# thourihan/DeepfakeDetection

Hardware: AMD Instinct MI355X
Metric: train images/sec @224^2 (EfficientNet-B0) (higher is better)
Workload: dtype bf16; 1 GPU; EfficientNet-b0 (timm flavour) 224x224 train step: bf16 fwd + label-smoothed CE + bwd + AdamW, random-init weights, 2 classes; per_gpu_batch=256, global_batch=256, parallelism=dp1, launch=hipgraph

## Files before the change

deepfakedetection_amd/_lib.py:

```python

from __future__ import annotations

import ctypes
from ctypes import POINTER, Structure, c_double, c_float, c_int, c_int64, c_long, c_size_t, c_uint32, c_void_p
from pathlib import Path

import os as _os

LIB_PATH = Path(_os.environ.get("DFD_LIB_PATH") or Path(__file__).resolve().parent / "libdfd_hip.so")

DFD_OK = 0
ERRORS = {-1: "DFD_EINVAL", -2: "DFD_EUNSUPPORTED", -3: "DFD_ELAUNCH", -4: "DFD_EWORKSPACE"}
F32, BF16 = 0, 1
ACT_NONE, ACT_SILU, ACT_RELU, ACT_GELU = 0, 1, 2, 3
PRO_NONE, PRO_BN_ACT, PRO_BN_ACT_GATE, PRO_AFFINE2 = 0, 1, 2, 3
MAX_PARTIALS = 1024
ADAMW_TABLE_COLS = 5
ADAMW_HP_LEN = 8
EMA_TABLE_COLS = 4
EMA_LERP, EMA_COPY = 0, 1
CLIP_MODE_NORM, CLIP_MODE_VALUE = 0, 1
CLIP_CFG_LEN = 2
CLIP_STATE_LEN = 8
(CLIP_NORM, CLIP_COEF, CLIP_SKIP, CLIP_STEPS, CLIP_CLIPPED, CLIP_SKIPPED, CLIP_NORM_SUM, CLIP_NORM_MAX) = range(8)
# ... 28 lines not shown


class StemShape(Structure):
    _fields_ = [(n, c_int) for n in ("N", "H", "W", "Cout", "Ho", "Wo", "k", "stride", "pad_top", "pad_left")]


class Mat(Structure):

    _fields_ = [(n, c_long) for n in ("sb", "sh", "sr", "sc")]


class Prologue(Structure):
    _fields_ = [
        ("mode", c_int), ("act", c_int), ("HW", c_int), ("_pad", c_int),
        ("a2", c_void_p), ("coef", c_void_p), ("gate", c_void_p),
    ]


P = c_void_p
_PI = POINTER(c_int)

SIGNATURES: dict[str, tuple] = {
    "dfd_version": (c_int, []),
    "dfd_tune": (c_int, [c_int, c_int]),
    "dfd_dw_mm_plan": (c_int, [POINTER(DwShape), c_int, _PI]),
    "dfd_bn_finalize": (c_int, [P, c_int, c_int, c_double, P, P, P, P, c_float, c_float, P, P]),
    "dfd_bn_eval_coeffs": (c_int, [P, P, P, P, c_float, c_int, P, P]),
    "dfd_bn_bwd_finalize": (c_int, [P, c_int, c_int, c_double, P, P, c_int, P, P, c_int, P, P]),
    "dfd_bn_act_apply": (c_int, [c_int, P, P, c_int, P, P, P, c_int, c_int, c_int, P]),
    "dfd_bn_bwd_reduce": (c_int, [c_int, P, P, P, P, c_int, c_int, c_int, P, c_int, _PI, P]),
    "dfd_gemm_bias_act": (c_int, [c_int, P, P, c_int, c_int, c_int, P, c_int, P, P, c_int, P, P, P]),
    "dfd_gemm_plan": (c_int, [c_int, c_int, c_int]),
    "dfd_pw_ntd_plan": (c_int, [c_int, c_int, c_int]),
    "dfd_bias_grad_ws": (c_size_t, [c_int, c_int, c_int]),
    "dfd_bias_grad": (c_int, [c_int, P, P, c_int, c_int, c_int, P, c_int, P, c_size_t, P]),
    "dfd_act_bn_bwd": (c_int, [c_int, P, P, P, P, P, c_int, P, c_int, c_int, c_int, P, c_int, _PI, P]),
    "dfd_act_bn_bwd_se": (c_int, [c_int, P, P, P, P, P, c_int, P, c_int, c_int, c_int, P, c_int, _PI, P, P, c_int, P, P, P, P, c_int, P]),
    "dfd_prep_weights_multi": (c_int, [P, c_int, P]),
    "dfd_resize_crop_u8": (c_int, [P, P, P, c_int, c_int, c_int, c_int, P]),
    "dfd_augment_u8": (c_int, [P, P, P, c_int, c_int, c_int, P]),
    "dfd_image_prep": (c_int, [P, P, c_int, c_int, c_int, POINTER(c_float), POINTER(c_float), P, P, P]),
    "dfd_pool_ws": (c_size_t, [c_int, c_int, c_int, c_int]),
    "dfd_pool_act": (c_int, [c_int, P, P, c_int, P, c_int, c_int, c_int, P, c_size_t, P]),
    "dfd_pool_bwd_reduce": (c_int, [c_int, P, P, P, c_int, P, c_int, c_int, c_int, P, c_size_t, P]),
    "dfd_scale_rows": (c_int, [c_int, P, P, P, c_int, c_int, c_int, P]),
    "dfd_se_fc_fwd": (c_int, [P, P, P, P, P, c_int, c_int, c_int, c_int, P, P, P, P]),
    "dfd_se_fc_bwd": (c_int, [P, P, P, P, P, P, c_int, c_int, c_int, c_int, P, P, P, P, P, c_int, P, P]),
    "dfd_dwconv_fwd": (c_int, [c_int, P, P, c_int, P, P, POINTER(DwShape), P, c_int, _PI, P]),
# ... 176 lines not shown
```

deepfakedetection_amd/csrc/dfd_pw.h:

```cpp
#pragma once
#include "dfd_common.h"
#include <type_traits>

typedef __attribute__((ext_vector_type(8))) __bf16 bf16x8_t;
typedef __attribute__((ext_vector_type(4))) short short4_t;
typedef __attribute__((ext_vector_type(8))) short short8_t;
typedef __attribute__((ext_vector_type(4))) float f32x4_t;

#define PW_BM 128

struct ProArgs {
    const void* a2;
    const float* coef;
    const float* gate;
    int HW;
    unsigned hw_magic;
    int hw_shift;
};
__device__ __forceinline__ int pro_image(const ProArgs& pa, int m) {
    return pa.hw_shift < 0 ? m : (int)(__umulhi((unsigned)m, pa.hw_magic) >> pa.hw_shift);
}

struct Magic { unsigned mul; int sh; };
static inline Magic make_magic(int d) {
    Magic m{0u, -1};
    if (d > 1) {
        int s = 0;
        while ((1ll << s) < d) ++s;
        m.mul = (unsigned)(((1ull << (31 + s)) + (unsigned long long)d - 1) / (unsigned long long)d);
        m.sh = s - 1;
    }
    return m;
// ... 104 lines not shown
        case DFD_ACT_SILU: { constexpr int ACT = DFD_ACT_SILU; __VA_ARGS__; } break; \
        case DFD_ACT_GELU: { constexpr int ACT = DFD_ACT_GELU; __VA_ARGS__; } break; \
        default: return DFD_EUNSUPPORTED;                                            \
    }
static inline bool pro_ok(const dfd_prologue* p) {
    if (!p) return true;
    switch (p->mode) {
        case DFD_PRO_NONE: return true;
        case DFD_PRO_BN_ACT: return p->coef != nullptr;
        case DFD_PRO_BN_ACT_GATE: return p->coef && p->gate && p->HW > 0;
        case DFD_PRO_AFFINE2: return p->coef && p->a2;
        default: return false;
    }
}
static inline ProArgs pro_args(const dfd_prologue* p) {
    ProArgs a{nullptr, nullptr, nullptr, 1, 0u, -1};
    if (p) { a.a2 = p->a2; a.coef = p->coef; a.gate = p->gate; a.HW = p->HW > 0 ? p->HW : 1; }
    if (a.HW > 1) {
        int sh = 0;
        while ((1ll << sh) < a.HW) ++sh;
        a.hw_magic = (unsigned)(((1ull << (31 + sh)) + (unsigned long long)a.HW - 1) / (unsigned long long)a.HW);
        a.hw_shift = sh - 1;
    }
    return a;
}


__device__ __forceinline__ int tn_off_bf16(int m, int ch) {
    const int f = ((m & 3) | (((m >> 3) & 1) << 2)) << 1;
    return m * 256 + ((ch ^ f) << 4);
}

// ... 18 lines not shown
```

deepfakedetection_amd/csrc/dfd_pwconv.hip:

```cpp
#include "dfd_pw.h"

template <typename T, int BN, int BM> struct NtLds {
    static constexpr int A_BYTES = BM * 128;
    static constexpr int B_BYTES = BN * 128;
    static constexpr int OROW = BN * (int)sizeof(T) + 16;
    static constexpr int OBYTES = BM * OROW;
    static constexpr int BOFF = ((2 * A_BYTES > OBYTES ? 2 * A_BYTES : OBYTES) + 15) / 16 * 16;
    static constexpr int TOTAL = BOFF + 2 * B_BYTES;
};

template <typename T, int BN, int BM, int PRO, int ACT, bool RES, bool STATS, bool CONV = false, int EACT = -1>
__global__ void __launch_bounds__(DFD_THREADS, 2)
k_pw_nt(const T* __restrict__ a, ProArgs pa, const T* __restrict__ w, T* __restrict__ out, const T* __restrict__ res,
        int M, int K, int Nout, int m_tiles, int n_tiles, int gx, float* __restrict__ partials, ConvArgs cv,
        const float* __restrict__ ebn = nullptr) {
    constexpr int E = El<T>::EPC;
    constexpr int BK = El<T>::BK;
    constexpr int NTW = BN / 32;
    using L = NtLds<T, BN, BM>;
    constexpr int RF = BM / 32;
    constexpr int AI = BM / 32;
    constexpr int OROW = L::OROW;
    extern __shared__ __attribute__((aligned(16))) unsigned char smem[];

// ... 771 lines not shown
    const bool small = ((M + 127) / 128) * ((Cout + 127) / 128) < 256;
#define CONV_GO(TT, BNV) return small ? conv_nt_launch<TT, BNV, 64>(x, s, in_bnstate, in_act, w_nk, y, Cout, partials, pcap, nparts, st) \
                                      : conv_nt_launch<TT, BNV, 128>(x, s, in_bnstate, in_act, w_nk, y, Cout, partials, pcap, nparts, st)
    if (dtype == DFD_BF16) { if (Cout <= 64) CONV_GO(bf16, 64); CONV_GO(bf16, 128); }
    if (dtype == DFD_F32) { if (Cout <= 64) CONV_GO(float, 64); CONV_GO(float, 128); }
#undef CONV_GO
    return DFD_EINVAL;
}

extern "C" int dfd_pwconv_fwd(int dtype, const void* a, const dfd_prologue* pro, const void* w, void* out,
                              const void* residual, int M, int K, int Nout, float* partials, int pcap, int* nparts,
                              dfd_stream stream) {
    if (!a || !w || !out || M < 1 || K < 8 || Nout < 8 || K % 8 || Nout % 8 || !pro_ok(pro)) return DFD_EINVAL;
    if (partials && (!nparts || pcap < 1)) return DFD_EINVAL;
    hipStream_t st = (hipStream_t)stream;
    const int rc = dfd_pw_ntw(dtype, a, pro, w, out, residual, M, K, Nout, partials, pcap, nparts, st);
    if (rc != DFD_EUNSUPPORTED) return rc;
    if (dtype == DFD_BF16 && !(!pro && !residual && !partials && dfd_gemm_plan(M, K, Nout))) {
        const int rd = dfd_pw_ntd(dtype, a, pro, w, out, residual, M, K, Nout, partials, pcap, nparts, st);
        if (rd != DFD_EUNSUPPORTED) return rd;
    }
    if (dtype == DFD_BF16) return pw_nt_t<bf16>(a, pro, w, out, residual, M, K, Nout, partials, pcap, nparts, st);
    if (dtype == DFD_F32) return pw_nt_t<float>(a, pro, w, out, residual, M, K, Nout, partials, pcap, nparts, st);
    return DFD_EINVAL;
}

extern "C" int dfd_pwconv_fwd_eval(int dtype, const void* a, const void* w, const float* out_bnstate, int out_act, void* out,
                                   int M, int K, int Nout, dfd_stream stream) {
    if (!a || !w || !out || !out_bnstate || M < 1 || K < 8 || Nout < 8 || K % 8 || Nout % 8) return DFD_EINVAL;
    hipStream_t st = (hipStream_t)stream;
// ... 148 lines not shown
```

deepfakedetection_amd/csrc/dfd_pwntd.hip:

```cpp
#include "dfd_pw.h"
#include "dfd_dwm.h"

#define ND_BM 64
#define ND_RED_BYTES (DFD_THREADS * 16 * 4)
#define ND_MAXN 192
#define ND_MINT 16

typedef __attribute__((address_space(3))) unsigned char nd_lds_u8;

__device__ __forceinline__ void nd_dma16(const void* src, unsigned lds_addr) {
    asm volatile("s_mov_b32 m0, %1\n\ts_nop 0\n\tglobal_load_lds_dwordx4 %0, off" : : "v"(src), "s"(lds_addr) : "memory");
}
template <int N> __device__ __forceinline__ void nd_wait_vm() { asm volatile("s_waitcnt vmcnt(%0)" : : "n"(N) : "memory"); }
__device__ __forceinline__ unsigned nd_lds_addr(const void* p) {
    return (unsigned)reinterpret_cast<uintptr_t>((nd_lds_u8*)p);
}

template <int NT, int PRO> struct NdGeom {
    static constexpr int BN = 16 * NT;
    static constexpr int WPC = (2 * NT + 3) / 4;
    static constexpr int JA = PRO == DFD_PRO_AFFINE2 ? 4 : 2;
    static constexpr int J = JA + WPC;
    static constexpr int WOFF = JA * 4096;
    static constexpr int STAGE = WOFF + WPC * 4096;
// ... 196 lines not shown
        float* red = reinterpret_cast<float*>(smem + (4 * 16 * OROW + 15) / 16 * 16);
        if (lact) {
            float* p = red + ((wave * RL + er) * CPR + ec) * 16;
            store_f32<8>(p, s1);
            store_f32<8>(p + 8, s2);
        }
        __syncthreads();
        for (int idx = t; idx < CPR * 16; idx += DFD_THREADS) {
            const int c = idx >> 4, x = idx & 15;
            float s = 0.f;
#pragma unroll 4
            for (int r = 0; r < 4 * RL; ++r) s += red[(r * CPR + c) * 16 + x];
            const int col = n0 + c * 8 + (x & 7);
            if (col < Nout) partials[(long)mt * 2 * Nout + (x >> 3) * Nout + col] = s;
        }
    }
}

template <int NT, int PRO, int ACT, bool RES, bool STATS>
static int ntd_launch(const void* a, const ProArgs& pa, const void* w, void* out, const void* residual, int M, int K, int Nout,
                      float* partials, int imgs, hipStream_t st) {
    using G = NdGeom<NT, PRO>;
    constexpr int NROW = PRO == DFD_PRO_AFFINE2 ? 3 : 2;
    const int m_tiles = (M + ND_BM - 1) / ND_BM, n_tiles = (Nout + G::BN - 1) / G::BN;
    const int nk = (K + 63) / 64;
    const int ctab = PRO == DFD_PRO_NONE ? 0 : (NROW * K * 4 + 1023) / 1024 * 1024 + 256;
    const int gtab = PRO == DFD_PRO_BN_ACT_GATE ? (imgs * K * 4 + 1023) / 1024 * 1024 + 256 : 0;
    const int tables = ctab + gtab;
    int ns;
    const int half = 80 * 1024 - 512;
// ... 34 lines not shown
    if (rc == DFD_OK && stats) *nparts = (M + ND_BM - 1) / ND_BM;
    return rc;
}

static int ntd_pick(int Nout) {
    const int tiles = (Nout + ND_MAXN - 1) / ND_MAXN;
    const int per = ((Nout + tiles - 1) / tiles + 15) / 16;
    return per <= 4 ? 4 : per <= 6 ? 6 : per <= 8 ? 8 : 12;
}

static bool ntd_serves(int M, int K, int cap) {
    const int m_tiles = (M + ND_BM - 1) / ND_BM;
    return (dfd_tune_get(DFD_TUNE_PW_NTD) & 1) && m_tiles >= ND_MINT && m_tiles <= cap && K >= 64 && (long)M * K < (1l << 30);
}

int dfd_pw_ntd(int dtype, const void* a, const dfd_prologue* pro, const void* w, void* out, const void* residual, int M, int K,
               int Nout, float* partials, int pcap, int* nparts, hipStream_t st) {
    const int cap = partials ? (pcap < DFD_MAX_PARTIALS ? pcap : DFD_MAX_PARTIALS) : DFD_MAX_PARTIALS;
    if (dtype != DFD_BF16 || !ntd_serves(M, K, cap)) return DFD_EUNSUPPORTED;
    switch (ntd_pick(Nout)) {
        case 4: return ntd_nt<4>(a, pro, w, out, residual, M, K, Nout, partials, nparts, st);
        case 6: return ntd_nt<6>(a, pro, w, out, residual, M, K, Nout, partials, nparts, st);
        case 8: return ntd_nt<8>(a, pro, w, out, residual, M, K, Nout, partials, nparts, st);
        default: return ntd_nt<12>(a, pro, w, out, residual, M, K, Nout, partials, nparts, st);
    }
}
extern "C" int dfd_pw_ntd_plan(int M, int K, int Nout) {
    return ntd_serves(M, K, DFD_MAX_PARTIALS) ? 16 * ntd_pick(Nout) : 0;
}
```

deepfakedetection_amd/csrc/dfd_pwntw.hip:

```cpp
#include "dfd_pw.h"

template <typename T, int BN, int KSN, int NCH, int PRO, int ACT, bool RES, bool STATS, int EACT = -1>
__global__ void __launch_bounds__(DFD_THREADS, 2)
k_pw_ntw(const T* __restrict__ a, ProArgs pa, const T* __restrict__ w, T* __restrict__ out, const T* __restrict__ res,
         int M, int K, int Nout, int m_tiles, int n_tiles, int gx, int wstride, int eoff, int coff, int nchunks,
         float* __restrict__ partials, const float* __restrict__ ebn = nullptr) {
    constexpr int E = El<T>::EPC;
    constexpr int BK = KSN * 4 * E;
    constexpr int JN = 4 / KSN;
    constexpr int WR = 16 * JN;
    constexpr int BM = 4 * WR;
    constexpr int NT = BN / 16;
    constexpr int OROW = BN * (int)sizeof(T) + 16;
    constexpr int CPR = BN / E;
    constexpr int RL = 64 / CPR;
    extern __shared__ __attribute__((aligned(16))) unsigned char smem[];

    const int total = gx * n_tiles;
    int lin = blockIdx.x;
    {
        const int q = total >> 3, r = total & 7, xcd = lin & 7, slot = lin >> 3;
        lin = (xcd < r ? xcd * (q + 1) : r * (q + 1) + (xcd - r) * q) + slot;
    }
    const int pb = lin / n_tiles, nt = lin - pb * n_tiles;
// ... 67 lines not shown
            const int rbase = mt * BM + wave * WR + frow;
#pragma unroll
            for (int j = 0; j < JN; ++j) {
                int row = rbase + j * 16;
                if (row >= M) row = M - 1;
                const float* grow = pa.gate + (long)pro_image(pa, row) * K;
#pragma unroll
                for (int ks = 0; ks < KSN; ++ks) {
                    int kk = kt * BK + (ks * 4 + fk) * E;
                    if (kk >= K) kk = 0;
                    load_f32<E>(grow + kk, gt[j][ks]);
                }
            }
        }
    };
    auto prologue = [&](const Regs& R, uint4 (&fa)[JN][KSN], int kt) {
        const float* cl = reinterpret_cast<const float*>(smem + coff);
        const int kp = nk * BK;
#pragma unroll
        for (int ks = 0; ks < KSN; ++ks)
#pragma unroll
            for (int j = 0; j < JN; ++j) {
                if constexpr (PRO == DFD_PRO_NONE) {
                    fa[j][ks] = (kt * BK + (ks * 4 + fk) * E < K) ? R.a[j][ks] : make_uint4(0, 0, 0, 0);
                } else {
                    const int kk = kt * BK + (ks * 4 + fk) * E;
                    float v[E], c0[E], c1[E];
                    load_f32<E>(cl + kk, c0);
                    load_f32<E>(cl + kp + kk, c1);
                    q_to_f(R.a[j][ks], v);
                    if constexpr (PRO == DFD_PRO_AFFINE2) {
                        float v2[E], c2[E];
                        load_f32<E>(cl + 2 * kp + kk, c2);
                        q_to_f(R.a2[j][ks], v2);
#pragma unroll
                        for (int x = 0; x < E; ++x) v[x] = fmaf(c0[x], v[x], fmaf(c1[x], v2[x], c2[x]));
                    } else {
                        bn_act_array<ACT, E>(v, c0, c1);
                        if constexpr (PRO == DFD_PRO_BN_ACT_GATE) {
#pragma unroll
                            for (int x = 0; x < E; ++x) v[x] = round_to<T>(v[x]) * gt[j][ks][x];
                        }
                    }
                    fa[j][ks] = kk < K ? f_to_q(v) : make_uint4(0, 0, 0, 0);
                }
            }
    };

    f32x4_t acc[NT][JN];
#pragma unroll
    for (int i = 0; i < NT; ++i)
#pragma unroll
        for (int j = 0; j < JN; ++j) acc[i][j] = (f32x4_t){0.f, 0.f, 0.f, 0.f};

    unsigned char* eb = smem + eoff + wave * WR * OROW;
    auto advance = [&](int& m_, int& k_) { if (++k_ == nk) { k_ = 0; m_ += gx; } };

    auto chunk = [&](const uint4 (&fa)[JN][KSN], int mt, int kt, int nc, float (&t1)[E], float (&t2)[E]) {
        {
// ... 96 lines not shown
                if (nc < nchunks) chunk(fa, mt, kt, nc, s1[nc], s2[nc]);
        } else {
            for (int nc = 0; nc < nchunks; ++nc) chunk(fa, mt, kt, nc, s1[0], s2[0]);
        }
    };

    int mt = pb, kt = 0;
    if (mt < m_tiles) {
        int mt1 = mt, kt1 = 0;
        advance(mt1, kt1);
        gate_load(mt, 0);
        g_load(R0, mt, 0);
        if (mt1 < m_tiles) g_load(R1, mt1, kt1);
        auto step = [&](Regs& rcur) -> bool {
            uint4 fa[JN][KSN];
            prologue(rcur, fa, kt);
            int mt2 = mt1, kt2 = kt1;
            advance(mt2, kt2);
            const bool has1 = mt1 < m_tiles;
            if (has1) {
                gate_load(mt1, kt1);
                if (mt2 < m_tiles) g_load(rcur, mt2, kt2);
            }
            compute(fa, mt, kt);
            if (!has1) return false;
            mt = mt1; kt = kt1;
            mt1 = mt2; kt1 = kt2;
            return true;
        };
        for (;;) {
            if (!step(R0)) break;
// ... 55 lines not shown
    if (panel > NTW_MAX_PANEL) return DFD_EUNSUPPORTED;
    const int coff = (panel + 15) / 16 * 16;
    const int eoff = coff + 3 * nk * BK * 4;
    constexpr int RED = DFD_THREADS * 2 * E * 4;
    int lds = eoff + 4 * WR * OROW;
    if (lds < RED) lds = RED;

    const int m_tiles = (M + BM - 1) / BM, n_tiles = (Nout + BN * nchunks - 1) / (BN * nchunks);
    const ProArgs pa = pro_args(pro);
    const int act = (pro && (mode == DFD_PRO_BN_ACT || mode == DFD_PRO_BN_ACT_GATE)) ? pro->act : DFD_ACT_NONE;
    const bool has_res = residual != nullptr;
    const int cap = partials ? (pcap < DFD_MAX_PARTIALS ? pcap : DFD_MAX_PARTIALS) : DFD_MAX_PARTIALS;

    if ((long)m_tiles * n_tiles < 1024 && nk * n_tiles > 2) return DFD_EUNSUPPORTED;

#define LAUNCH_NTW_(NCHV, PRO, RES, STATS)                                                                                      \
    do {                                                                                                                  \
        auto kern = k_pw_ntw<T, BN, KSN, NCHV, PRO, ACT, RES, STATS>;                                                        \
        int gx = (256 * ntw_blocks_per_cu(kern, lds)) / n_tiles;                                                          \
        if (gx < 32) gx = 32;                                                                                             \
        if (gx > cap) gx = cap;                                                                                           \
        if (gx > m_tiles) gx = m_tiles;                                                                                   \
        if (partials) *nparts = gx;                                                                                       \
        hipLaunchKernelGGL(kern, dim3(gx * n_tiles), dim3(DFD_THREADS), lds, st, (const T*)a, pa, (const T*)w, (T*)out,   \
                           (const T*)residual, M, K, Nout, m_tiles, n_tiles, gx, wstride, eoff, coff, nchunks, partials,  \
                           (const float*)nullptr);                                                                        \
    } while (0)
#define LAUNCH_NTW(PRO, RES, STATS) LAUNCH_NTW_(1, PRO, RES, STATS)
    if (ebn) {
        if (mode != DFD_PRO_NONE || has_res || stats || eact != DFD_ACT_SILU) return DFD_EUNSUPPORTED;
        auto kern = k_pw_ntw<T, BN, KSN, 1, DFD_PRO_NONE, DFD_ACT_NONE, false, false, DFD_ACT_SILU>;
        int gx = (256 * ntw_blocks_per_cu(kern, lds)) / n_tiles;
        if (gx < 32) gx = 32;
        if (gx > cap) gx = cap;
        if (gx > m_tiles) gx = m_tiles;
        hipLaunchKernelGGL(kern, dim3(gx * n_tiles), dim3(DFD_THREADS), lds, st, (const T*)a, pa, (const T*)w, (T*)out,
                           (const T*)nullptr, M, K, Nout, m_tiles, n_tiles, gx, wstride, eoff, coff, nchunks, (float*)nullptr, ebn);
        return DFD_CHECK_LAUNCH();
    }
    if (mode == DFD_PRO_AFFINE2) {
        constexpr int ACT = DFD_ACT_NONE;
        if (stats) return DFD_EUNSUPPORTED;
        if (has_res) LAUNCH_NTW(DFD_PRO_AFFINE2, true, false); else LAUNCH_NTW(DFD_PRO_AFFINE2, false, false);
    } else if (mode == DFD_PRO_NONE) {
        constexpr int ACT = DFD_ACT_NONE;
        if (has_res && stats) return DFD_EUNSUPPORTED;
        if (has_res) LAUNCH_NTW(DFD_PRO_NONE, true, false);
        else if (stats) LAUNCH_NTW(DFD_PRO_NONE, false, true);
        else LAUNCH_NTW(DFD_PRO_NONE, false, false);
    } else {
        if (has_res) return DFD_EUNSUPPORTED;
        if (mode == DFD_PRO_BN_ACT) {
            DISPATCH_ACT_PW(act, { if (stats) LAUNCH_NTW(DFD_PRO_BN_ACT, false, true); else LAUNCH_NTW(DFD_PRO_BN_ACT, false, false); });
        } else {
            DISPATCH_ACT_PW(act, { if (stats) LAUNCH_NTW(DFD_PRO_BN_ACT_GATE, false, true); else LAUNCH_NTW(DFD_PRO_BN_ACT_GATE, false, false); });
        }
    }
#undef LAUNCH_NTW
// ... 27 lines not shown
```

deepfakedetection_amd/csrc/dfd_rowpass.hip:

```cpp
#include "dfd_common.h"
#include "dfd_se.h"
#include "dfd_sum.h"

template <typename T, int ACT, bool HAS_RES, bool HAS_RS>
__global__ void __launch_bounds__(DFD_THREADS)
k_bn_act_apply(const T* __restrict__ y, const float* __restrict__ bnstate, const T* __restrict__ res,
               const float* __restrict__ rs, T* __restrict__ out, long total_vec, int CV, int C, long vec_per_img) {
    constexpr int V = Vec<T>::N;
    const long stride = (long)gridDim.x * DFD_THREADS;
    const long first = (long)blockIdx.x * DFD_THREADS + threadIdx.x;
    int cv = (int)(first % CV);
    const int cstep = (int)(stride % CV);
    for (long i = first; i < total_vec; i += stride, cv = cv + cstep >= CV ? cv + cstep - CV : cv + cstep) {
        const int c0 = cv * V;
        float v[V], sc[V], sh[V];
        Vec<T>::load(y + i * V, v);
        load_f32<V>(bnstate + c0, sc);
        load_f32<V>(bnstate + C + c0, sh);
        float r = 1.f;
        if constexpr (HAS_RS) r = rs[i / vec_per_img];
        float q[V];
        if constexpr (HAS_RES) Vec<T>::load(res + i * V, q);
        bn_act_array<ACT, V>(v, sc, sh);
#pragma unroll
// ... 667 lines not shown
                                      dfd_stream stream) {
    if (!partials || nparts < 1 || C < 1 || count <= 0 || !bnstate || !coef) return DFD_EINVAL;
    if (dls && (!ls_gamma || !beta)) return DFD_EINVAL;
    const int threads = FIN_CH * FIN_LANES, grid = (C + FIN_CH - 1) / FIN_CH;
    hipLaunchKernelGGL(k_bn_bwd_finalize, dim3(grid), dim3(threads), 0, (hipStream_t)stream, partials, nparts, C, count,
                       gamma, beta, ls_gamma, bnstate, train, dgamma, dbeta, dls, dbias, accumulate, coef);
    return DFD_CHECK_LAUNCH();
}
extern "C" int dfd_bn_bwd_finalize(const float* partials, int nparts, int C, double count, const float* gamma,
                                   const float* bnstate, int train, float* dgamma, float* dbeta, int accumulate,
                                   float* coef, dfd_stream stream) {
    return dfd_bn_bwd_finalize_ex(partials, nparts, C, count, gamma, nullptr, nullptr, bnstate, train, dgamma, dbeta, nullptr,
                                  nullptr, accumulate, coef, stream);
}

extern "C" int dfd_version(void) { return 150; }
```

deepfakedetection_amd/functions.py:

```python

from __future__ import annotations

import contextlib
import os
import threading
from dataclasses import dataclass

import torch

from . import kernels as K
from ._lib import ACT_NONE, ACT_SILU
from .arch import ConvGeom
from .arena import grad_dest


@dataclass
class BNRef:

    running_mean: torch.Tensor
    running_var: torch.Tensor
    num_batches_tracked: torch.Tensor | None
    momentum: float
    eps: float

# ... 257 lines not shown
    def backward(ctx, g):
        cfg: MBConvCtx = ctx.cfg
        x, y1, y2, y3, st1, st2, st3, pooled, hpre, gate, wexp_kn, wproj_kn, w2t, *t, row_scale = ctx.saved_tensors
        need = ctx.needs_input_grad
        exp, dw, proj, se = _mb_layers(t, need[1:], cfg)
        tr = cfg.training
        geom = cfg.dw
        N, H, W, Cin = x.shape
        _, Ho, Wo, Cmid = y2.shape
        g = _c(g)
        gb = K.scale_rows(g, row_scale) if ctx.has_rs else g
        parts, n = K.bn_bwd_reduce(gb, y3, st3, None)
        Cout, R = y3.shape[3], se[0].shape[0]
        w1 = se[0].reshape(R, -1)
        coef3 = bn_backward(proj, parts, n, N * Ho * Wo, st3, tr)
        gm3 = K.affine2_apply(gb, y3, coef3)
        D, _, _ = K.pwconv(gm3, None, wproj_kn, None, stats=False)
        if proj.need_w:
            pro_q = K.pro_bn_act_gate(st2, ACT_SILU, gate, Ho * Wo)
            proj.dw = K.pwconv_wgrad(gm3, None, y2, pro_q, _slot(proj.w, True, (Cout, Cmid))).view(Cout, Cmid, 1, 1)
        need_se = need[7:11]
        se_outs = tuple(_slot(p, nd, shape) for p, nd, shape in zip(se, need_se, ((R, Cmid), (R,), (Cmid, R), (Cmid,))))
        se_res = K.se_bwd(D, y2, st2, ACT_SILU, gate, hpre, pooled, w1, w2t, ACT_SILU, any(need_se), se_outs, defer_wgrad=True)
        dpooled, dw1, db1, dw2, db2 = se_res[:5]
        se_job = se_res[5]
        dz2, parts, n = K.act_bn_bwd(D, y2, gate, dpooled, st2, ACT_SILU, se_job=se_job)
        if dw1 is not None:
            dw1, dw2 = dw1.view(dw1.shape[0], -1, 1, 1), dw2.view(dw2.shape[0], -1, 1, 1)
        coef2 = bn_backward(dw, parts, n, N * Ho * Wo, st2, tr)
        dx = None
        if cfg.expand:
            dz1, parts, n = K.dwconv_bwd_data(dz2, y2, coef2, dw.w, y1, st1, ACT_SILU, y1.shape, geom.kernel,
# ... 162 lines not shown
```

deepfakedetection_amd/kernels.py:

```python

from __future__ import annotations

import contextlib
import functools
import ctypes
import math
import threading
import weakref
from dataclasses import dataclass

import os

import torch

from . import _lib
from ._lib import (
    ACT_NONE, ACT_SILU, BF16, CLIP_CFG_LEN, CLIP_STATE_LEN, F32, MAX_PARTIALS, MIX_CUTMIX, MIX_JOB_WORDS, MIX_KEEP, MIX_NCHW, MIX_NHWC, PRO_AFFINE2, PRO_BN_ACT,
    PRO_BN_ACT_GATE, PRO_NONE, DwShape, Prologue, StemShape, check,
)

_scratch: dict[tuple[int, int, str], torch.Tensor] = {}


def _L():
# ... 817 lines not shown
    if isinstance(w_nk, MxWeight):
        if residual is not None or stats:
            raise ValueError("the MX fp8 GEMM has no residual / statistics epilogue")
        aq, asc = mx_quant_rows(a, pro)
        return mx_gemm(aq, asc, w_nk, a.dtype, (*a.shape[:-1], w_nk.N)), None, 0
    K = a.shape[-1]
    M = a.numel() // K
    Nout = w_nk.shape[0]
    out = torch.empty((*a.shape[:-1], Nout), dtype=a.dtype, device=a.device)
    parts = partials_buf(a.device, Nout) if stats else None
    n = ctypes.c_int(0)
    check(_L().dfd_pwconv_fwd(_dt(a), _p(a), ctypes.byref(pro) if pro is not None else None, _p(w_nk), _p(out),
                              _p(residual), M, K, Nout, _p(parts), MAX_PARTIALS, ctypes.byref(n), _stream()),
          "dfd_pwconv_fwd", f"M={M} K={K} N={Nout}")
    return out, parts, n.value


def pwconv_eval(a: torch.Tensor, w_nk: torch.Tensor, out_state: torch.Tensor, out_act: int) -> torch.Tensor:
    K = a.shape[-1]
    M = a.numel() // K
    Nout = w_nk.shape[0]
    out = torch.empty((*a.shape[:-1], Nout), dtype=a.dtype, device=a.device)
    check(_L().dfd_pwconv_fwd_eval(_dt(a), _p(a), _p(w_nk), _p(out_state), out_act, _p(out), M, K, Nout, _stream()),
          "dfd_pwconv_fwd_eval", f"M={M} K={K} N={Nout}")
    return out


def dwconv_eval(x: torch.Tensor, w: torch.Tensor, out_state: torch.Tensor, out_act: int, k: int, stride: int, pad_top: int,
                pad_left: int, Ho: int, Wo: int):
    _chk_nhwc(x)
# ... 955 lines not shown
```

include/dfd_hip.h:

```cpp
#ifndef DFD_HIP_H
#define DFD_HIP_H

#include <stddef.h>
#include <stdint.h>

#ifdef __cplusplus
extern "C" {
#endif

typedef void* dfd_stream;

#define DFD_OK            0
#define DFD_EINVAL       (-1)
#define DFD_EUNSUPPORTED (-2)
#define DFD_ELAUNCH      (-3)
#define DFD_EWORKSPACE   (-4)

#define DFD_F32   0
#define DFD_BF16  1

#define DFD_ACT_NONE 0
#define DFD_ACT_SILU 1
#define DFD_ACT_RELU 2
#define DFD_ACT_GELU 3
// ... 43 lines not shown
int dfd_bn_bwd_finalize_ex(const float* partials, int nparts, int C, double count, const float* gamma,
                           const float* beta, const float* ls_gamma, const float* bnstate, int train,
                           float* dgamma, float* dbeta, float* dls, float* dbias, int accumulate,
                           float* coef, dfd_stream stream);

int dfd_bn_act_apply(int dtype, const void* y, const float* bnstate, int act,
                     const void* residual, const float* row_scale, void* out,
                     int N, int HW, int C, dfd_stream stream);
int dfd_bn_bwd_reduce(int dtype, const void* g, const void* y, const float* bnstate,
                      const float* row_scale, int N, int HW, int C,
                      float* partials, int pcap, int* nparts, dfd_stream stream);
int dfd_gemm_bias_act(int dtype, const void* a, const void* w_nk, int M, int K, int N, const float* state, int act,
                      const void* residual, const float* row_scale, int HW, void* yraw, void* out, dfd_stream stream);
int dfd_gemm_plan(int M, int K, int N);
int dfd_pw_ntd_plan(int M, int K, int Nout);
size_t dfd_bias_grad_ws(int N, int HW, int C);
int dfd_bias_grad(int dtype, const void* g, const float* row_scale, int N, int HW, int C, float* dbias, int accumulate,
                  float* ws, size_t ws_bytes, dfd_stream stream);
int dfd_act_bn_bwd(int dtype, const void* D, const void* y, const float* gate,
                   const float* dpool, const float* bnstate, int act, void* dz,
                   int N, int HW, int C, float* partials, int pcap, int* nparts,
                   dfd_stream stream);
int dfd_act_bn_bwd_se(int dtype, const void* D, const void* y, const float* gate, const float* dpool,
                      const float* bnstate, int act, void* dz, int N, int HW, int C, float* partials, int pcap,
                      int* nparts, const float* se_pooled, const float* se_ws, int R, float* dw1, float* db1, float* dw2,
                      float* db2, int accumulate, dfd_stream stream);
size_t dfd_pool_ws(int dtype, int N, int HW, int C);
int dfd_pool_act(int dtype, const void* y, const float* bnstate, int act, float* pooled,
                 int N, int HW, int C, void* ws, size_t ws_bytes, dfd_stream stream);
int dfd_pool_bwd_reduce(int dtype, const void* D, const void* y, const float* bnstate,
// ... 50 lines not shown
                     float* w2t, dfd_stream stream);
size_t dfd_dwconv_bwd_weight_ws(const dfd_dwconv_shape* s);

#define DFD_PRO_NONE        0
#define DFD_PRO_BN_ACT      1
#define DFD_PRO_BN_ACT_GATE 2
#define DFD_PRO_AFFINE2     3
typedef struct {
    int mode;
    int act;
    int HW;
    int _pad;
    const void* a2;
    const float* coef;
    const float* gate;
} dfd_prologue;

int dfd_pwconv_fwd(int dtype, const void* a, const dfd_prologue* pro, const void* w,
                   void* out, const void* residual, int M, int K, int Nout,
                   float* partials, int pcap, int* nparts, dfd_stream stream);
int dfd_pwconv_wgrad(int dtype, const void* p, const dfd_prologue* pro_p, int Ni,
                     const void* q, const dfd_prologue* pro_q, int Nj, int M,
                     float* dw, int accumulate, float* ws, size_t ws_bytes,
                     dfd_stream stream);
int dfd_pwconv_bwd_fused(int dtype, const void* dz, const void* y, const float* coef, const void* x, const void* w_kn,
                         const void* residual, int M, int Cm, int Cin, void* dx, float* dw, int accumulate, float* ws,
                         size_t ws_bytes, dfd_stream stream);
size_t dfd_pwconv_wgrad_ws(int M, int Ni, int Nj);
int dfd_pw_prep_weights(int dtype, const float* w, void* w_nk, void* w_kn, int N, int K,
                        dfd_stream stream);
// ... 295 lines not shown
```

Baseline: 20780 images/sec.

## Fuse affine2 backward prologue into projection-conv data-grad GEMM with side output

In the MBConv projection backward, the separate affine2_apply kernel and the following pwconv are replaced by one GEMM launch. That launch applies the AFFINE2 prologue in registers and also writes the mapped gradient gm3 out as a side tensor for the later weight-grad. A new sweep kernel (k_pw_nts) keeps the A tile resident in registers and sweeps a few N tiles. The ntw path also gains a SIDE template variant. This removes one elementwise pass over the activation and one re-read of it, at the cost of more kernel variants and a fallback path when the shape is unsupported.

```diff
diff --git a/deepfakedetection_amd/_lib.py b/deepfakedetection_amd/_lib.py
--- a/deepfakedetection_amd/_lib.py
+++ b/deepfakedetection_amd/_lib.py
@@ -66,6 +66,7 @@
     _fields_ = [
         ("mode", c_int), ("act", c_int), ("HW", c_int), ("_pad", c_int),
         ("a2", c_void_p), ("coef", c_void_p), ("gate", c_void_p),
+        ("side", c_void_p),
     ]
 
 
@@ -84,6 +85,7 @@
     "dfd_gemm_bias_act": (c_int, [c_int, P, P, c_int, c_int, c_int, P, c_int, P, P, c_int, P, P, P]),
     "dfd_gemm_plan": (c_int, [c_int, c_int, c_int]),
     "dfd_pw_ntd_plan": (c_int, [c_int, c_int, c_int]),
+    "dfd_pw_ntd_sweep_plan": (c_int, [c_int, c_int, c_int]),
     "dfd_bias_grad_ws": (c_size_t, [c_int, c_int, c_int]),
     "dfd_bias_grad": (c_int, [c_int, P, P, c_int, c_int, c_int, P, c_int, P, c_size_t, P]),
     "dfd_act_bn_bwd": (c_int, [c_int, P, P, P, P, P, c_int, P, c_int, c_int, c_int, P, c_int, _PI, P]),
diff --git a/deepfakedetection_amd/csrc/dfd_pw.h b/deepfakedetection_amd/csrc/dfd_pw.h
--- a/deepfakedetection_amd/csrc/dfd_pw.h
+++ b/deepfakedetection_amd/csrc/dfd_pw.h
@@ -16,6 +16,7 @@
     int HW;
     unsigned hw_magic;
     int hw_shift;
+    void* side;
 };
 __device__ __forceinline__ int pro_image(const ProArgs& pa, int m) {
     return pa.hw_shift < 0 ? m : (int)(__umulhi((unsigned)m, pa.hw_magic) >> pa.hw_shift);
@@ -150,8 +151,9 @@
     }
 }
 static inline ProArgs pro_args(const dfd_prologue* p) {
-    ProArgs a{nullptr, nullptr, nullptr, 1, 0u, -1};
+    ProArgs a{nullptr, nullptr, nullptr, 1, 0u, -1, nullptr};
     if (p) { a.a2 = p->a2; a.coef = p->coef; a.gate = p->gate; a.HW = p->HW > 0 ? p->HW : 1; }
+    if (p && p->mode == DFD_PRO_AFFINE2) a.side = p->side;
     if (a.HW > 1) {
         int sh = 0;
         while ((1ll << sh) < a.HW) ++sh;
diff --git a/deepfakedetection_amd/csrc/dfd_pwconv.hip b/deepfakedetection_amd/csrc/dfd_pwconv.hip
--- a/deepfakedetection_amd/csrc/dfd_pwconv.hip
+++ b/deepfakedetection_amd/csrc/dfd_pwconv.hip
@@ -809,6 +809,13 @@
     if (!a || !w || !out || M < 1 || K < 8 || Nout < 8 || K % 8 || Nout % 8 || !pro_ok(pro)) return DFD_EINVAL;
     if (partials && (!nparts || pcap < 1)) return DFD_EINVAL;
     hipStream_t st = (hipStream_t)stream;
+    if (pro && pro->side) {
+        if (pro->mode != DFD_PRO_AFFINE2) return DFD_EINVAL;
+        if (dtype != DFD_BF16 || partials) return DFD_EUNSUPPORTED;
+        const int rw = dfd_pw_ntw(dtype, a, pro, w, out, residual, M, K, Nout, partials, pcap, nparts, st);
+        if (rw != DFD_EUNSUPPORTED) return rw;
+        return dfd_pw_ntd(dtype, a, pro, w, out, residual, M, K, Nout, partials, pcap, nparts, st);
+    }
     const int rc = dfd_pw_ntw(dtype, a, pro, w, out, residual, M, K, Nout, partials, pcap, nparts, st);
     if (rc != DFD_EUNSUPPORTED) return rc;
     if (dtype == DFD_BF16 && !(!pro && !residual && !partials && dfd_gemm_plan(M, K, Nout))) {
diff --git a/deepfakedetection_amd/csrc/dfd_pwntd.hip b/deepfakedetection_amd/csrc/dfd_pwntd.hip
--- a/deepfakedetection_amd/csrc/dfd_pwntd.hip
+++ b/deepfakedetection_amd/csrc/dfd_pwntd.hip
@@ -234,6 +234,154 @@
             const int col = n0 + c * 8 + (x & 7);
             if (col < Nout) partials[(long)mt * 2 * Nout + (x >> 3) * Nout + col] = s;
         }
+    }
+}
+
+#define NS_MAXK 320
+#define NS_SLOTS 512
+#define NS_MAXSWEEP 2
+
+template <int NT> struct NsGeom {
+    static constexpr int BN = 16 * NT;
+    static constexpr int WPC = (2 * NT + 3) / 4;
+    static constexpr int STAGE = WPC * 4096;
+    static constexpr int OROW = BN * 2 + 16;
+    static constexpr int EPI = (4 * 16 * OROW + 15) / 16 * 16;
+};
+
+template <int NT, int KS>
+__global__ void __launch_bounds__(DFD_THREADS, 2)
+k_pw_nts(const unsigned short* __restrict__ a, ProArgs pa, const unsigned short* __restrict__ w, unsigned short* __restrict__ out,
+         int M, int K, int Nout, int m_tiles, int n_tiles, int cgroups, int ns, int eoff) {
+    using G = NsGeom<NT>;
+    constexpr int BN = G::BN, WPC = G::WPC, J = G::WPC, OROW = G::OROW;
+    static_assert(KS % 2 == 0, "whole 64-wide K steps");
+    extern __shared__ __attribute__((aligned(16))) unsigned char smem[];
+
+    const int total = m_tiles * cgroups;
+    int lin = blockIdx.x;
+    {
+        const int q = total >> 3, r = total & 7, xcd = lin & 7, slot = lin >> 3;
+        lin = (xcd < r ? xcd * (q + 1) : r * (q + 1) + (xcd - r) * q) + slot;
+    }
+    const int mt = lin / cgroups, cg = lin - mt * cgroups;
+    const int c0 = cg * n_tiles / cgroups, c1 = (cg + 1) * n_tiles / cgroups;
+    const int m0 = mt * ND_BM;
+    const int t = threadIdx.x, lane = t & 63;
+    const int wave = __builtin_amdgcn_readfirstlane(t >> 6);
+    const int frow = lane & 15, fk = lane >> 4;
+    const int nk = (K + 63) >> 6;
+    const int S = (c1 - c0) * nk;
+    const unsigned lds0 = nd_lds_addr(smem);
+
+    uint4 fa[KS];
+    {
+        const int row = m0 + wave * 16 + frow;
+        const long rbase = (long)(row < M ? row : M - 1) * K;
+        const unsigned short* a2 = reinterpret_cast<const unsigned short*>(pa.a2);
+        uint4 ra2[KS];
+#pragma unroll
+        for (int g = 0; g < KS; ++g) {
+            const int kk = g * 32 + fk * 8;
+            const long off = rbase + (kk < K ? kk : 0);
+            fa[g] = *reinterpret_cast<const uint4*>(a + off);
+            ra2[g] = *reinterpret_cast<const uint4*>(a2 + off);
+        }
+#pragma unroll
+        for (int g = 0; g < KS; ++g) {
+            const int kk = g * 32 + fk * 8;
+            const int kc = kk < K ? kk : 0;
+            float c0v[8], c1v[8], c2v[8], gt[8];
+            load_f32<8>(pa.coef + kc, c0v);
+            load_f32<8>(pa.coef + K + kc, c1v);
+            load_f32<8>(pa.coef + 2 * K + kc, c2v);
+#pragma unroll
+            for (int x = 0; x < 8; ++x) gt[x] = 0.f;
+            fa[g] = apply_pro_v<bf16, DFD_PRO_AFFINE2, DFD_ACT_NONE, 8>(fa[g], ra2[g], c0v, c1v, c2v, gt);
+            if (cg == 0 && row < M && kk < K)
+                *reinterpret_cast<uint4*>(reinterpret_cast<unsigned short*>(pa.side) + rbase + kk) = fa[g];
+            if (kk >= K) fa[g] = make_uint4(0, 0, 0, 0);
+        }
+    }
+
+    const int cs = (lane & 7) ^ ((lane >> 3) & 7);
+    int rq_n0 = c0 * BN, rq_kt = 0;
+    auto request = [&](int buf) {
+        int k = rq_kt * 64 + cs * 8;
+        if (k >= K) k = K - 8;
+        const unsigned sb = lds0 + buf * G::STAGE + wave * 1024;
+        const char* wb = reinterpret_cast<const char*>(w) + k * 2;
+#pragma unroll
+        for (int j = 0; j < WPC; ++j) {
+            const int r = rq_n0 + (j * 4 + wave) * 8 + (lane >> 3);
+            const int n = r < Nout ? r : Nout - 1;
+            nd_dma16(wb + (unsigned)n * (unsigned)K * 2u, sb + j * 4096);
+        }
+        if (++rq_kt == nk) { rq_kt = 0; rq_n0 += BN; }
+    };
+    const int D = ns - 1;
+    for (int s = 0; s < D && s < S; ++s) request(s);
+
+    unsigned char* eb = smem + eoff + wave * 16 * OROW;
+    constexpr int CPR = BN / 8;
+    constexpr int RL = 64 / CPR;
+    constexpr int NPS = (16 + RL - 1) / RL;
+    const int ec = lane % CPR, er = lane / CPR;
+    const bool lact = er < RL;
+    const int mw = m0 + wave * 16;
+
+    int buf = 0, s = 0;
+    for (int nt = c0; nt < c1; ++nt) {
+        const int n0 = nt * BN;
+        f32x4_t acc[NT];
+#pragma unroll
+        for (int i = 0; i < NT; ++i) acc[i] = (f32x4_t){0.f, 0.f, 0.f, 0.f};
+#pragma unroll
+        for (int kt = 0; kt < KS / 2; ++kt) {
+            if (kt < nk) {
+                const int ahead = S - 1 - s < D - 1 ? S - 1 - s : D - 1;
+                if (ahead >= 2) nd_wait_vm<2 * J>();
+                else if (ahead == 1) nd_wait_vm<J>();
+                else nd_wait_vm<0>();
+                __syncthreads();
+                if (s + D < S) {
+                    int nb = buf + D;
+                    if (nb >= ns) nb -= ns;
+                    request(nb);
+                }
+                const unsigned char* sw = smem + buf * G::STAGE;
+#pragma unroll
+                for (int ks = 0; ks < 2; ++ks) {
+                    const int sl = ((ks * 4 + fk) ^ (frow & 7)) << 4;
+                    uint4 fw[NT];
+#pragma unroll
+                    for (int i = 0; i < NT; ++i) fw[i] = *reinterpret_cast<const uint4*>(sw + (i * 16 + frow) * 128 + sl);
+                    __builtin_amdgcn_sched_barrier(0);
+#pragma unroll
+                    for (int i = 0; i < NT; ++i)
+                        acc[i] = __builtin_amdgcn_mfma_f32_16x16x32_bf16(__builtin_bit_cast(bf16x8_t, fw[i]),
+                                                                         __builtin_bit_cast(bf16x8_t, fa[kt * 2 + ks]), acc[i], 0, 0, 0);
+                }
+                if (++buf == ns) buf = 0;
+                ++s;
+            }
+        }
+
+#pragma unroll
+        for (int i = 0; i < NT; ++i)
+            *reinterpret_cast<uint2*>(eb + frow * OROW + (i * 16 + fk * 4) * 2) = make_uint2(pack_bf2(acc[i][0], acc[i][1]), pack_bf2(acc[i][2], acc[i][3]));
+        __builtin_amdgcn_fence(__ATOMIC_RELEASE, "wavefront");
+        __builtin_amdgcn_wave_barrier();
+        __builtin_amdgcn_fence(__ATOMIC_ACQUIRE, "wavefront");
+        const int n = n0 + ec * 8;
+#pragma unroll
+        for (int u = 0; u < NPS; ++u) {
+            const int r = er + u * RL, m = mw + r;
+            if (lact && r < 16 && m < M && n < Nout)
+                *reinterpret_cast<uint4*>(out + (long)m * Nout + n) = *reinterpret_cast<const uint4*>(eb + r * OROW + ec * 16);
+        }
+        __builtin_amdgcn_fence(__ATOMIC_RELEASE, "wavefront");
+        __builtin_amdgcn_wave_barrier();
     }
 }
 
@@ -298,10 +446,55 @@
     return (dfd_tune_get(DFD_TUNE_PW_NTD) & 1) && m_tiles >= ND_MINT && m_tiles <= cap && K >= 64 && (long)M * K < (1l << 30);
 }
 
+static int nts_groups(int M, int K, int Nout) {
+    const int n_tiles = (Nout + 16 * ntd_pick(Nout) - 1) / (16 * ntd_pick(Nout));
+    if (K > NS_MAXK || n_tiles < 2) return 0;
+    const int m_tiles = (M + ND_BM - 1) / ND_BM;
+    const int groups = 2 * m_tiles <= NS_SLOTS ? 2 : 1;
+    return (n_tiles + groups - 1) / groups <= NS_MAXSWEEP ? groups : 0;
+}
+
+template <int NT, int KS>
+static int nts_launch(const void* a, const ProArgs& pa, const void* w, void* out, int M, int K, int Nout, hipStream_t st) {
+    using G = NsGeom<NT>;
+    const int m_tiles = (M + ND_BM - 1) / ND_BM, n_tiles = (Nout + G::BN - 1) / G::BN;
+    const int nk = (K + 63) / 64;
+    const int cgroups = nts_groups(M, K, Nout);
+    int ns;
+    const int half = 80 * 1024 - 512;
+    if (3 * G::STAGE + G::EPI <= half) ns = 3;
+    else if (2 * G::STAGE + G::EPI <= half) ns = 2;
+    else { ns = (160 * 1024 - 1024 - G::EPI) / G::STAGE; if (ns > 4) ns = 4; }
+    const int stages = (n_tiles + cgroups - 1) / cgroups * nk;
+    if (ns > stages + 1) ns = stages + 1;
+    if (ns < 2) ns = 2;
+    const int ring = ns * G::STAGE;
+    const int lds = ring + G::EPI;
+    if (lds > 160 * 1024 || 2 * nk > KS) return DFD_EUNSUPPORTED;
+    constexpr auto kern = k_pw_nts<NT, KS>;
+    dfd_allow_lds_once<kern>(160 * 1024);
+    hipLaunchKernelGGL(kern, dim3((unsigned)(m_tiles * cgroups)), dim3(DFD_THREADS), lds, st, (const unsigned short*)a, pa,
+                       (const unsigned short*)w, (unsigned short*)out, M, K, Nout, m_tiles, n_tiles, cgroups, ns, ring);
+    return DFD_CHECK_LAUNCH();
+}
+
+template <int NT>
+static int nts_nt(const void* a, const ProArgs& pa, const void* w, void* out, int M, int K, int Nout, hipStream_t st) {
+    const int nk = (K + 63) / 64;
+    if (nk <= 2) return nts_launch<NT, 4>(a, pa, w, out, M, K, Nout, st);
+    if (nk <= 3) return nts_launch<NT, 6>(a, pa, w, out, M, K, Nout, st);
+    return nts_launch<NT, 10>(a, pa, w, out, M, K, Nout, st);
+}
+
 int dfd_pw_ntd(int dtype, const void* a, const dfd_prologue* pro, const void* w, void* out, const void* residual, int M, int K,
                int Nout, float* partials, int pcap, int* nparts, hipStream_t st) {
     const int cap = partials ? (pcap < DFD_MAX_PARTIALS ? pcap : DFD_MAX_PARTIALS) : DFD_MAX_PARTIALS;
     if (dtype != DFD_BF16 || !ntd_serves(M, K, cap)) return DFD_EUNSUPPORTED;
+    if (pro && pro->side) {
+        if (pro->mode != DFD_PRO_AFFINE2 || residual || partials || !nts_groups(M, K, Nout)) return DFD_EUNSUPPORTED;
+        const ProArgs pa = pro_args(pro);
+        return ntd_pick(Nout) == 8 ? nts_nt<8>(a, pa, w, out, M, K, Nout, st) : nts_nt<12>(a, pa, w, out, M, K, Nout, st);
+    }
     switch (ntd_pick(Nout)) {
         case 4: return ntd_nt<4>(a, pro, w, out, residual, M, K, Nout, partials, nparts, st);
         case 6: return ntd_nt<6>(a, pro, w, out, residual, M, K, Nout, partials, nparts, st);
@@ -312,3 +505,6 @@
 extern "C" int dfd_pw_ntd_plan(int M, int K, int Nout) {
     return ntd_serves(M, K, DFD_MAX_PARTIALS) ? 16 * ntd_pick(Nout) : 0;
 }
+extern "C" int dfd_pw_ntd_sweep_plan(int M, int K, int Nout) {
+    return ntd_serves(M, K, DFD_MAX_PARTIALS) ? nts_groups(M, K, Nout) : 0;
+}
diff --git a/deepfakedetection_amd/csrc/dfd_pwntw.hip b/deepfakedetection_amd/csrc/dfd_pwntw.hip
--- a/deepfakedetection_amd/csrc/dfd_pwntw.hip
+++ b/deepfakedetection_amd/csrc/dfd_pwntw.hip
@@ -1,6 +1,6 @@
 #include "dfd_pw.h"
 
-template <typename T, int BN, int KSN, int NCH, int PRO, int ACT, bool RES, bool STATS, int EACT = -1>
+template <typename T, int BN, int KSN, int NCH, int PRO, int ACT, bool RES, bool STATS, int EACT = -1, bool SIDE = false>
 __global__ void __launch_bounds__(DFD_THREADS, 2)
 k_pw_ntw(const T* __restrict__ a, ProArgs pa, const T* __restrict__ w, T* __restrict__ out, const T* __restrict__ res,
          int M, int K, int Nout, int m_tiles, int n_tiles, int gx, int wstride, int eoff, int coff, int nchunks,
@@ -105,7 +105,7 @@
             }
         }
     };
-    auto prologue = [&](const Regs& R, uint4 (&fa)[JN][KSN], int kt) {
+    auto prologue = [&](const Regs& R, uint4 (&fa)[JN][KSN], int mt_, int kt) {
         const float* cl = reinterpret_cast<const float*>(smem + coff);
         const int kp = nk * BK;
 #pragma unroll
@@ -134,6 +134,11 @@
                         }
                     }
                     fa[j][ks] = kk < K ? f_to_q(v) : make_uint4(0, 0, 0, 0);
+                    if constexpr (SIDE && PRO == DFD_PRO_AFFINE2) {
+                        const int row = mt_ * BM + wave * WR + frow + j * 16;
+                        if (row < M && kk < K)
+                            *reinterpret_cast<uint4*>(reinterpret_cast<T*>(pa.side) + (long)row * K + kk) = fa[j][ks];
+                    }
                 }
             }
     };
@@ -260,7 +265,7 @@
         if (mt1 < m_tiles) g_load(R1, mt1, kt1);
         auto step = [&](Regs& rcur) -> bool {
             uint4 fa[JN][KSN];
-            prologue(rcur, fa, kt);
+            prologue(rcur, fa, mt, kt);
             int mt2 = mt1, kt2 = kt1;
             advance(mt2, kt2);
             const bool has1 = mt1 < m_tiles;
@@ -346,9 +351,9 @@
 
     if ((long)m_tiles * n_tiles < 1024 && nk * n_tiles > 2) return DFD_EUNSUPPORTED;
 
-#define LAUNCH_NTW_(NCHV, PRO, RES, STATS)                                                                                      \
+#define LAUNCH_NTW_(NCHV, PRO, RES, STATS, SIDEV)                                                                               \
     do {                                                                                                                  \
-        auto kern = k_pw_ntw<T, BN, KSN, NCHV, PRO, ACT, RES, STATS>;                                                        \
+        auto kern = k_pw_ntw<T, BN, KSN, NCHV, PRO, ACT, RES, STATS, -1, SIDEV>;                                             \
         int gx = (256 * ntw_blocks_per_cu(kern, lds)) / n_tiles;                                                          \
         if (gx < 32) gx = 32;                                                                                             \
         if (gx > cap) gx = cap;                                                                                           \
@@ -358,7 +363,7 @@
                            (const T*)residual, M, K, Nout, m_tiles, n_tiles, gx, wstride, eoff, coff, nchunks, partials,  \
                            (const float*)nullptr);                                                                        \
     } while (0)
-#define LAUNCH_NTW(PRO, RES, STATS) LAUNCH_NTW_(1, PRO, RES, STATS)
+#define LAUNCH_NTW(PRO, RES, STATS) LAUNCH_NTW_(1, PRO, RES, STATS, false)
     if (ebn) {
         if (mode != DFD_PRO_NONE || has_res || stats || eact != DFD_ACT_SILU) return DFD_EUNSUPPORTED;
         auto kern = k_pw_ntw<T, BN, KSN, 1, DFD_PRO_NONE, DFD_ACT_NONE, false, false, DFD_ACT_SILU>;
@@ -373,7 +378,10 @@
     if (mode == DFD_PRO_AFFINE2) {
         constexpr int ACT = DFD_ACT_NONE;
         if (stats) return DFD_EUNSUPPORTED;
-        if (has_res) LAUNCH_NTW(DFD_PRO_AFFINE2, true, false); else LAUNCH_NTW(DFD_PRO_AFFINE2, false, false);
+        if (pa.side) {
+            if (has_res || n_tiles > 1) return DFD_EUNSUPPORTED;
+            LAUNCH_NTW_(1, DFD_PRO_AFFINE2, false, false, true);
+        } else if (has_res) LAUNCH_NTW(DFD_PRO_AFFINE2, true, false); else LAUNCH_NTW(DFD_PRO_AFFINE2, false, false);
     } else if (mode == DFD_PRO_NONE) {
         constexpr int ACT = DFD_ACT_NONE;
         if (has_res && stats) return DFD_EUNSUPPORTED;
diff --git a/deepfakedetection_amd/csrc/dfd_rowpass.hip b/deepfakedetection_amd/csrc/dfd_rowpass.hip
--- a/deepfakedetection_amd/csrc/dfd_rowpass.hip
+++ b/deepfakedetection_amd/csrc/dfd_rowpass.hip
@@ -705,4 +705,4 @@
                                   nullptr, accumulate, coef, stream);
 }
 
-extern "C" int dfd_version(void) { return 150; }
+extern "C" int dfd_version(void) { return 151; }
diff --git a/deepfakedetection_amd/functions.py b/deepfakedetection_amd/functions.py
--- a/deepfakedetection_amd/functions.py
+++ b/deepfakedetection_amd/functions.py
@@ -295,8 +295,7 @@
         Cout, R = y3.shape[3], se[0].shape[0]
         w1 = se[0].reshape(R, -1)
         coef3 = bn_backward(proj, parts, n, N * Ho * Wo, st3, tr)
-        gm3 = K.affine2_apply(gb, y3, coef3)
-        D, _, _ = K.pwconv(gm3, None, wproj_kn, None, stats=False)
+        D, gm3 = K.pwconv_mapped(gb, y3, coef3, wproj_kn)
         if proj.need_w:
             pro_q = K.pro_bn_act_gate(st2, ACT_SILU, gate, Ho * Wo)
             proj.dw = K.pwconv_wgrad(gm3, None, y2, pro_q, _slot(proj.w, True, (Cout, Cmid))).view(Cout, Cmid, 1, 1)
diff --git a/deepfakedetection_amd/kernels.py b/deepfakedetection_amd/kernels.py
--- a/deepfakedetection_amd/kernels.py
+++ b/deepfakedetection_amd/kernels.py
@@ -855,6 +855,33 @@
                               _p(residual), M, K, Nout, _p(parts), MAX_PARTIALS, ctypes.byref(n), _stream()),
           "dfd_pwconv_fwd", f"M={M} K={K} N={Nout}")
     return out, parts, n.value
+
+
+def pwconv_mapped(g: torch.Tensor, y: torch.Tensor, coef: torch.Tensor, w_nk: torch.Tensor, fused: bool = True):
+    if fused and not isinstance(w_nk, MxWeight) and g.dtype == torch.bfloat16:
+        K = g.shape[-1]
+        M = g.numel() // K
+        Nout = w_nk.shape[0]
+        gm = torch.empty_like(y)
+        out = torch.empty((*g.shape[:-1], Nout), dtype=g.dtype, device=g.device)
+        pro = pro_affine2(y, coef)
+        pro.side = _p(gm)
+        sink = _profile_sink
+        if sink is not None:
+            e0, e1 = torch.cuda.Event(enable_timing=True), torch.cuda.Event(enable_timing=True)
+            e0.record()
+        n = ctypes.c_int(0)
+        rc = _L().dfd_pwconv_fwd(_dt(g), _p(g), ctypes.byref(pro), _p(w_nk), _p(out), None, M, K, Nout, None, MAX_PARTIALS,
+                                 ctypes.byref(n), _stream())
+        if rc != _UNSUPPORTED:
+            check(rc, "dfd_pwconv_fwd", f"mapped M={M} K={K} N={Nout}")
+            if sink is not None:
+                e1.record()
+                nbytes = _tensor_bytes((g, y, coef, w_nk, out, gm))
+                sink.append(("pwconv", nbytes, 2.0 * M * K * Nout, e0, e1, _bytes_8d("pwconv", (g, None, w_nk), nbytes)))
+            return out, gm
+    gm = affine2_apply(g, y, coef)
+    return pwconv(gm, None, w_nk, None, stats=False)[0], gm
 
 
 def pwconv_eval(a: torch.Tensor, w_nk: torch.Tensor, out_state: torch.Tensor, out_act: int) -> torch.Tensor:
diff --git a/include/dfd_hip.h b/include/dfd_hip.h
--- a/include/dfd_hip.h
+++ b/include/dfd_hip.h
@@ -81,6 +81,7 @@
                       const void* residual, const float* row_scale, int HW, void* yraw, void* out, dfd_stream stream);
 int dfd_gemm_plan(int M, int K, int N);
 int dfd_pw_ntd_plan(int M, int K, int Nout);
+int dfd_pw_ntd_sweep_plan(int M, int K, int Nout);
 size_t dfd_bias_grad_ws(int N, int HW, int C);
 int dfd_bias_grad(int dtype, const void* g, const float* row_scale, int N, int HW, int C, float* dbias, int accumulate,
                   float* ws, size_t ws_bytes, dfd_stream stream);
@@ -161,6 +162,7 @@
     const void* a2;
     const float* coef;
     const float* gate;
+    void* side;
 } dfd_prologue;
 
 int dfd_pwconv_fwd(int dtype, const void* a, const dfd_prologue* pro, const void* w,
```

Result: no change. 20880 images/sec, median of 6 (+0.5%).
